# NVIDIA-Merlin/distributed-embeddings

Measured on AMD Instinct MI355X. Metric: samples/sec (whole node) DLRM-Criteo-1TB bs/gpu=65536, higher is better.
Workload: dtype bf16; 1 GPU; model=DLRM-Criteo-1TB, global_batch=65536, batch_per_gpu=65536, embedding_dim=128, parallelism=hybrid dp+mp (strategy=memory_balanced) x1

## Files before the change

distributed_embeddings_amd/csrc/dot_interact.hip:

```cpp

#include <hip/hip_runtime.h>
#include <hip/hip_bf16.h>

#include "ops_api.h"

#define WAVE 64

typedef __attribute__((ext_vector_type(8))) short bf16x8;
typedef __attribute__((ext_vector_type(4))) float f32x4;


template <int FMAX>
__global__ void dot_interact_fwd(const __hip_bfloat16* __restrict__ feats,
                                 __hip_bfloat16* __restrict__ out, int64_t B,
                                 int F, int D, int out_w, int tri_n) {
  extern __shared__ short lds_all[];
  const int wave = threadIdx.x >> 6;
  const int lane = threadIdx.x & (WAVE - 1);
  const int ldst = D + 8;
  short* lds = lds_all + wave * FMAX * ldst;
  const int64_t n_waves = ((int64_t)gridDim.x * blockDim.x) >> 6;
  const int64_t wave_id = ((int64_t)blockIdx.x * blockDim.x + threadIdx.x) >> 6;

  for (int64_t b = wave_id; b < B; b += n_waves) {
    const short* src = reinterpret_cast<const short*>(feats) + b * (int64_t)F * D;
    const int total8 = FMAX * D / 8;
    for (int i = lane; i < total8; i += WAVE) {
      const int elem = i * 8;
      const int row = elem / D, col = elem % D;
      if (elem < F * D) {
        *reinterpret_cast<bf16x8*>(&lds[row * ldst + col]) =
            *reinterpret_cast<const bf16x8*>(&src[elem]);
      } else {
        bf16x8 z = {0, 0, 0, 0, 0, 0, 0, 0};
        *reinterpret_cast<bf16x8*>(&lds[row * ldst + col]) = z;
      }
    }

    const int r16 = lane & 15;
    const int khalf = lane >> 4;

    const int tiles_mi[3] = {0, 1, 1};
    const int tiles_ni[3] = {0, 0, 1};
#pragma unroll
    for (int t = 0; t < 3; ++t) {
      const int mi = tiles_mi[t], ni = tiles_ni[t];
      f32x4 acc = {0.f, 0.f, 0.f, 0.f};
      for (int k0 = 0; k0 < D; k0 += 32) {
        bf16x8 a = *reinterpret_cast<const bf16x8*>(
            &lds[(mi * 16 + r16) * ldst + k0 + khalf * 8]);
        bf16x8 bfr = *reinterpret_cast<const bf16x8*>(
            &lds[(ni * 16 + r16) * ldst + k0 + khalf * 8]);
        acc = __builtin_amdgcn_mfma_f32_16x16x32_bf16(a, bfr, acc, 0, 0, 0);
      }
      __hip_bfloat16* orow = out + b * (int64_t)out_w;
#pragma unroll
      for (int reg = 0; reg < 4; ++reg) {
        const int i = mi * 16 + (lane >> 4) * 4 + reg;
        const int j = ni * 16 + (lane & 15);
        if (i > j && i < F && j < F) {
          orow[i * (i - 1) / 2 + j] = __hip_bfloat16(acc[reg]);
        }
      }
    }
    short* orow_s = reinterpret_cast<short*>(out + b * (int64_t)out_w);
    for (int c = lane; c < D; c += WAVE) {
      orow_s[tri_n + c] = lds[c];
    }
    for (int c = tri_n + D + lane; c < out_w; c += WAVE) {
      orow_s[c] = 0;
    }
  }
}

template <int FMAX>
__global__ void dot_interact_bwd(const __hip_bfloat16* __restrict__ gout,
                                 const __hip_bfloat16* __restrict__ feats,
                                 __hip_bfloat16* __restrict__ gfeats, int64_t B,
                                 int F, int D, int out_w, int tri_n) {
  extern __shared__ short lds_all[];
  const int wave = threadIdx.x >> 6;
  const int lane = threadIdx.x & (WAVE - 1);
  short* lds = lds_all + wave * (FMAX * D + FMAX * FMAX);
  short* gsym = lds + FMAX * D;
  const int64_t n_waves = ((int64_t)gridDim.x * blockDim.x) >> 6;
  const int64_t wave_id = ((int64_t)blockIdx.x * blockDim.x + threadIdx.x) >> 6;

  for (int64_t b = wave_id; b < B; b += n_waves) {
    const short* src = reinterpret_cast<const short*>(feats) + b * (int64_t)F * D;
    const int total8 = FMAX * D / 8;
    for (int i = lane; i < total8; i += WAVE) {
      const int elem = i * 8;
      if (elem < F * D) {
        *reinterpret_cast<bf16x8*>(&lds[elem]) =
            *reinterpret_cast<const bf16x8*>(&src[elem]);
      } else {
        bf16x8 z = {0, 0, 0, 0, 0, 0, 0, 0};
        *reinterpret_cast<bf16x8*>(&lds[elem]) = z;
      }
    }
    const __hip_bfloat16* grow = gout + b * (int64_t)out_w;
    for (int idx = lane; idx < FMAX * FMAX; idx += WAVE) {
      const int i = idx / FMAX, j = idx % FMAX;
      float g = 0.f;
      if (i < F && j < F && i != j) {
        const int r = i > j ? i : j, c = i > j ? j : i;
        g = float(grow[r * (r - 1) / 2 + c]);
      }
      __hip_bfloat16 hb(g);
      gsym[idx] = *reinterpret_cast<short*>(&hb);
    }

    const int r16 = lane & 15;
    const int khalf = lane >> 4;
    __hip_bfloat16* gf = gfeats + b * (int64_t)F * D;

    for (int nj = 0; nj < D / 16; ++nj) {
#pragma unroll
      for (int mi = 0; mi < FMAX / 16; ++mi) {
        f32x4 acc = {0.f, 0.f, 0.f, 0.f};
#pragma unroll
        for (int k0 = 0; k0 < FMAX; k0 += 32) {
          bf16x8 a = *reinterpret_cast<const bf16x8*>(
              &gsym[(mi * 16 + r16) * FMAX + k0 + khalf * 8]);
          bf16x8 bfr;
#pragma unroll
          for (int r = 0; r < 8; ++r) {
            bfr[r] = lds[(k0 + khalf * 8 + r) * D + nj * 16 + r16];
          }
          acc = __builtin_amdgcn_mfma_f32_16x16x32_bf16(a, bfr, acc, 0, 0, 0);
        }
#pragma unroll
        for (int reg = 0; reg < 4; ++reg) {
          const int i = mi * 16 + (lane >> 4) * 4 + reg;
          const int j = nj * 16 + (lane & 15);
          if (i < F && j < D) {
            float v = acc[reg];
            if (i == 0) v += float(grow[tri_n + j]);
            gf[i * D + j] = __hip_bfloat16(v);
          }
        }
      }
    }
  }
}



static int di_wpb(int dflt) {
  static int v = [] {
    const char* e = getenv("DE_DI_WPB");
    if (!e) return 0;
    int i = atoi(e);
    return (i == 2 || i == 4 || i == 8) ? i : 0;
  }();
  return v ? v : dflt;
}

template <int FMAX, int WPB>
__global__ void dot_interact_fwd_packed(
    const __hip_bfloat16* __restrict__ bottom,
    const __hip_bfloat16* __restrict__ packed,
    const int* __restrict__ perm, __hip_bfloat16* __restrict__ out, int64_t B,
    int F, int D, int out_w, int tri_n, int64_t sb, int64_t sp) {
  extern __shared__ short lds_all[];
  const int wave = threadIdx.x >> 6;
  const int lane = threadIdx.x & (WAVE - 1);
  const int tid = threadIdx.x;
  const int ldst = D + 8;
  short* lds = lds_all + wave * FMAX * ldst;
  const int d8 = D / 8;

  for (int64_t b0 = (int64_t)blockIdx.x * WPB; b0 < B;
       b0 += (int64_t)gridDim.x * WPB) {
    for (int i = tid; i < FMAX * WPB * d8; i += WPB * WAVE) {
      const int row = i / (WPB * d8);
      const int rem = i % (WPB * d8);
      const int w = rem / d8;
      const int col = (rem % d8) * 8;
      const int64_t b = b0 + w;
      bf16x8 v = {0, 0, 0, 0, 0, 0, 0, 0};
      if (b < B) {
        if (row == 0) {
          v = *reinterpret_cast<const bf16x8*>(
              reinterpret_cast<const short*>(bottom) + b * (int64_t)D + col);
        } else if (row < F) {
          v = *reinterpret_cast<const bf16x8*>(
              reinterpret_cast<const short*>(packed) +
              ((int64_t)perm[row - 1] * sp + b * sb) * (int64_t)D + col);
        }
      }
      *reinterpret_cast<bf16x8*>(
          &lds_all[w * FMAX * ldst + row * ldst + col]) = v;
    }
    __syncthreads();

    const int64_t b = b0 + wave;
    if (b < B) {
      const int r16 = lane & 15;
      const int khalf = lane >> 4;
      const int tiles_mi[3] = {0, 1, 1};
      const int tiles_ni[3] = {0, 0, 1};
#pragma unroll
      for (int t = 0; t < 3; ++t) {
        const int mi = tiles_mi[t], ni = tiles_ni[t];
        f32x4 acc = {0.f, 0.f, 0.f, 0.f};
        for (int k0 = 0; k0 < D; k0 += 32) {
          bf16x8 a = *reinterpret_cast<const bf16x8*>(
              &lds[(mi * 16 + r16) * ldst + k0 + khalf * 8]);
          bf16x8 bfr = *reinterpret_cast<const bf16x8*>(
              &lds[(ni * 16 + r16) * ldst + k0 + khalf * 8]);
          acc = __builtin_amdgcn_mfma_f32_16x16x32_bf16(a, bfr, acc, 0, 0, 0);
        }
        __hip_bfloat16* orow = out + b * (int64_t)out_w;
#pragma unroll
        for (int reg = 0; reg < 4; ++reg) {
          const int i = mi * 16 + (lane >> 4) * 4 + reg;
          const int j = ni * 16 + (lane & 15);
          if (i > j && i < F && j < F) {
            orow[i * (i - 1) / 2 + j] = __hip_bfloat16(acc[reg]);
          }
        }
      }
      short* orow_s = reinterpret_cast<short*>(out + b * (int64_t)out_w);
      for (int c = lane; c < D; c += WAVE) {
        orow_s[tri_n + c] = lds[c];
      }
      for (int c = tri_n + D + lane; c < out_w; c += WAVE) {
        orow_s[c] = 0;
      }
    }
    __syncthreads();
  }
}

template <int FMAX, int WPB>
__global__ void dot_interact_bwd_packed(
    const __hip_bfloat16* __restrict__ gout,
    const __hip_bfloat16* __restrict__ bottom,
    const __hip_bfloat16* __restrict__ packed, const int* __restrict__ perm,
    __hip_bfloat16* __restrict__ gbottom, __hip_bfloat16* __restrict__ gpacked,
    int64_t B, int F, int D, int out_w, int tri_n, int64_t sb, int64_t sp) {
  extern __shared__ short lds_all[];
  const int wave = threadIdx.x >> 6;
  const int lane = threadIdx.x & (WAVE - 1);
  const int tid = threadIdx.x;
  const int per_wave = FMAX * D + FMAX * FMAX;
  short* lds = lds_all + wave * per_wave;
  short* gsym = lds + FMAX * D;
  const int d8 = D / 8;

  for (int64_t b0 = (int64_t)blockIdx.x * WPB; b0 < B;
       b0 += (int64_t)gridDim.x * WPB) {
    for (int i = tid; i < FMAX * WPB * d8; i += WPB * WAVE) {
      const int row = i / (WPB * d8);
      const int rem = i % (WPB * d8);
      const int w = rem / d8;
      const int col = (rem % d8) * 8;
      const int64_t b = b0 + w;
      bf16x8 v = {0, 0, 0, 0, 0, 0, 0, 0};
      if (b < B) {
        if (row == 0) {
          v = *reinterpret_cast<const bf16x8*>(
              reinterpret_cast<const short*>(bottom) + b * (int64_t)D + col);
        } else if (row < F) {
          v = *reinterpret_cast<const bf16x8*>(
              reinterpret_cast<const short*>(packed) +
              ((int64_t)perm[row - 1] * sp + b * sb) * (int64_t)D + col);
        }
      }
      *reinterpret_cast<bf16x8*>(
          &lds_all[w * per_wave + row * D + col]) = v;
    }
    __syncthreads();

    const int64_t b = b0 + wave;
    if (b < B) {
      const __hip_bfloat16* grow = gout + b * (int64_t)out_w;
      for (int idx = lane; idx < FMAX * FMAX; idx += WAVE) {
        const int i = idx / FMAX, j = idx % FMAX;
        float g = 0.f;
        if (i < F && j < F && i != j) {
          const int r = i > j ? i : j, c = i > j ? j : i;
          g = float(grow[r * (r - 1) / 2 + c]);
        }
        __hip_bfloat16 hb(g);
        gsym[idx] = *reinterpret_cast<short*>(&hb);
      }

      const int r16 = lane & 15;
      const int khalf = lane >> 4;
      for (int nj = 0; nj < D / 16; ++nj) {
        f32x4 accs[FMAX / 16];
#pragma unroll
        for (int mi = 0; mi < FMAX / 16; ++mi) {
          f32x4 acc = {0.f, 0.f, 0.f, 0.f};
#pragma unroll
          for (int k0 = 0; k0 < FMAX; k0 += 32) {
            bf16x8 a = *reinterpret_cast<const bf16x8*>(
                &gsym[(mi * 16 + r16) * FMAX + k0 + khalf * 8]);
            bf16x8 bfr;
#pragma unroll
            for (int r = 0; r < 8; ++r) {
              bfr[r] = lds[(k0 + khalf * 8 + r) * D + nj * 16 + r16];
            }
            acc = __builtin_amdgcn_mfma_f32_16x16x32_bf16(a, bfr, acc, 0, 0, 0);
          }
          accs[mi] = acc;
        }
#pragma unroll
        for (int mi = 0; mi < FMAX / 16; ++mi) {
#pragma unroll
          for (int reg = 0; reg < 4; ++reg) {
            const int i = mi * 16 + (lane >> 4) * 4 + reg;
            const int j = nj * 16 + (lane & 15);
            float v = accs[mi][reg];
            if (i == 0) v += float(grow[tri_n + j]);
            __hip_bfloat16 hb(v);
            lds[i * D + j] = *reinterpret_cast<short*>(&hb);
          }
        }
      }
    }
    __syncthreads();

    for (int i = tid; i < FMAX * WPB * d8; i += WPB * WAVE) {
      const int row = i / (WPB * d8);
      const int rem = i % (WPB * d8);
      const int w = rem / d8;
      const int col = (rem % d8) * 8;
      const int64_t b = b0 + w;
      if (b >= B || row >= F) continue;
      const bf16x8 v = *reinterpret_cast<const bf16x8*>(
          &lds_all[w * per_wave + row * D + col]);
      if (row == 0) {
        *reinterpret_cast<bf16x8*>(
            reinterpret_cast<short*>(gbottom) + b * (int64_t)D + col) = v;
      } else {
        *reinterpret_cast<bf16x8*>(
            reinterpret_cast<short*>(gpacked) +
            ((int64_t)perm[row - 1] * sp + b * sb) * (int64_t)D + col) = v;
      }
    }
    __syncthreads();
  }
}

void launch_dot_interact_fwd_packed(const void* bottom, const void* packed,
                                    const int* perm, void* out, int64_t B,
                                    int F, int D, int out_w, int tri_n,
                                    int64_t sb, int64_t sp,
                                    hipStream_t stream) {
  const int wpb = di_wpb(2);
  const int block = wpb * WAVE;
  int64_t blocks = (B + wpb - 1) / wpb;
  if (blocks > 32768) blocks = 32768;
  const size_t lds = (size_t)wpb * 32 * (D + 8) * sizeof(short);
#define LFWD(W)                                                                \
  hipLaunchKernelGGL((dot_interact_fwd_packed<32, W>), dim3((int)blocks),      \
                     dim3(block), lds, stream,                                 \
                     (const __hip_bfloat16*)bottom,                            \
                     (const __hip_bfloat16*)packed, perm, (__hip_bfloat16*)out,\
                     B, F, D, out_w, tri_n, sb, sp)
  if (wpb == 2) LFWD(2); else if (wpb == 8) LFWD(8); else LFWD(4);
#undef LFWD
}

void launch_dot_interact_bwd_packed(const void* gout, const void* bottom,
                                    const void* packed, const int* perm,
                                    void* gbottom, void* gpacked, int64_t B,
                                    int F, int D, int out_w, int tri_n,
                                    int64_t sb, int64_t sp,
                                    hipStream_t stream) {
  const int wpb = di_wpb(8);
  const int block = wpb * WAVE;
  int64_t blocks = (B + wpb - 1) / wpb;
  if (blocks > 32768) blocks = 32768;
  const size_t lds = (size_t)wpb * (32 * D + 32 * 32) * sizeof(short);
#define LBWD(W)                                                                \
  hipLaunchKernelGGL((dot_interact_bwd_packed<32, W>), dim3((int)blocks),      \
                     dim3(block), lds, stream, (const __hip_bfloat16*)gout,    \
                     (const __hip_bfloat16*)bottom,                            \
                     (const __hip_bfloat16*)packed, perm,                      \
                     (__hip_bfloat16*)gbottom, (__hip_bfloat16*)gpacked, B, F, \
                     D, out_w, tri_n, sb, sp)
  if (wpb == 2) LBWD(2); else if (wpb == 8) LBWD(8); else LBWD(4);
#undef LBWD
}

void launch_dot_interact_fwd(const void* feats, void* out, int64_t B, int F,
                             int D, int out_w, int tri_n, hipStream_t stream) {
  const int block = 256;
  const int waves = block / WAVE;
  int64_t blocks = (B + waves - 1) / waves;
  if (blocks > 8192) blocks = 8192;
  const size_t lds = (size_t)waves * 32 * (D + 8) * sizeof(short);
  hipLaunchKernelGGL((dot_interact_fwd<32>), dim3((int)blocks), dim3(block),
                     lds, stream, (const __hip_bfloat16*)feats,
                     (__hip_bfloat16*)out, B, F, D, out_w, tri_n);
}

void launch_dot_interact_bwd(const void* gout, const void* feats, void* gfeats,
                             int64_t B, int F, int D, int out_w, int tri_n,
                             hipStream_t stream) {
  const int block = 256;
  const int waves = block / WAVE;
  int64_t blocks = (B + waves - 1) / waves;
  if (blocks > 8192) blocks = 8192;
  const size_t lds = (size_t)waves * (32 * D + 32 * 32) * sizeof(short);
  hipLaunchKernelGGL((dot_interact_bwd<32>), dim3((int)blocks), dim3(block),
                     lds, stream, (const __hip_bfloat16*)gout,
                     (const __hip_bfloat16*)feats, (__hip_bfloat16*)gfeats, B,
                     F, D, out_w, tri_n);
}
```

Baseline: 16.32 million samples/s.

## Specialize packed dot-interaction kernels on compile-time embedding dim with MFMA tile restructuring

Adds D-templated forward and backward packed dot-interaction kernels, used when D is 32, 64, 128 or 256. They precompute gather offsets per thread, launch one block per group instead of grid-striding, and compute only the three needed lower-triangular 16x16 tiles in forward. Forward stages each output row in LDS so it can be written with vectorized stores. Backward uses swizzled LDS, transposed LDS reads (ds_read_tr16) and per-wave fences in place of block barriers. Default waves per block change to 4 for both directions. The cost is added code complexity, larger register use from the unrolled offset arrays, and a fallback path only for unsupported D.

```diff
diff --git a/distributed_embeddings_amd/csrc/dot_interact.hip b/distributed_embeddings_amd/csrc/dot_interact.hip
--- a/distributed_embeddings_amd/csrc/dot_interact.hip
+++ b/distributed_embeddings_amd/csrc/dot_interact.hip
@@ -147,6 +147,8 @@
 
 
 
+#define DI_WPB_FWD 4
+#define DI_WPB_BWD 4
 static int di_wpb(int dflt) {
   static int v = [] {
     const char* e = getenv("DE_DI_WPB");
@@ -158,7 +160,7 @@
 }
 
 template <int FMAX, int WPB>
-__global__ void dot_interact_fwd_packed(
+__global__ void dot_interact_fwd_packed_rt(
     const __hip_bfloat16* __restrict__ bottom,
     const __hip_bfloat16* __restrict__ packed,
     const int* __restrict__ perm, __hip_bfloat16* __restrict__ out, int64_t B,
@@ -235,7 +237,7 @@
 }
 
 template <int FMAX, int WPB>
-__global__ void dot_interact_bwd_packed(
+__global__ void dot_interact_bwd_packed_rt(
     const __hip_bfloat16* __restrict__ gout,
     const __hip_bfloat16* __restrict__ bottom,
     const __hip_bfloat16* __restrict__ packed, const int* __restrict__ perm,
@@ -346,23 +348,355 @@
   }
 }
 
+
+typedef __attribute__((ext_vector_type(4))) short bf16x4;
+typedef bf16x8 __attribute__((aligned(2))) bf16x8_u;
+typedef short v4i16_t __attribute__((vector_size(8)));
+typedef __attribute__((address_space(3))) v4i16_t lds_v4i16_t;
+
+__device__ __forceinline__ void wave_lds_fence() {
+  __builtin_amdgcn_fence(__ATOMIC_ACQ_REL, "wavefront");
+  __builtin_amdgcn_wave_barrier();
+}
+
+__device__ __forceinline__ short f32_to_bf16_bits(float v) {
+  __hip_bfloat16 hb(v);
+  return *reinterpret_cast<short*>(&hb);
+}
+
+__device__ __forceinline__ float bf16_bits_to_f32(short s) {
+  return __builtin_bit_cast(float, (unsigned)(unsigned short)s << 16);
+}
+
+template <int D>
+__device__ __forceinline__ int swz(int row, int col) {
+  const int sw = (((row & 3) << 2) | ((row >> 2) & 3)) & (D / 8 - 1);
+  return row * D + ((((col >> 3) ^ sw) << 3) | (col & 7));
+}
+
+template <int D, int WPB>
+struct PackedIO {
+  static constexpr int D8 = D / 8;
+  static constexpr int RPI = WAVE / D8;
+  static constexpr int NIT = 32 / RPI;
+  int r0, w, col;
+  int64_t b;
+  int64_t off[NIT];
+
+  __device__ __forceinline__ PackedIO(const int* __restrict__ perm, int F,
+                                      int64_t b0, int64_t sb, int64_t sp) {
+    const int tid = threadIdx.x;
+    r0 = tid / (WPB * D8);
+    w = (tid / D8) % WPB;
+    col = (tid % D8) * 8;
+    b = b0 + w;
+    int prow[NIT];
+#pragma unroll
+    for (int it = 0; it < NIT; ++it) {
+      const int row = it * RPI + r0;
+      const int pi = row < 1 ? 0 : (row < F ? row - 1 : F - 2);
+      prow[it] = perm[pi];
+    }
+#pragma unroll
+    for (int it = 0; it < NIT; ++it) {
+      const int row = it * RPI + r0;
+      off[it] = row == 0 ? b * D + col
+                         : (prow[it] * sp + b * sb) * (int64_t)D + col;
+    }
+#pragma unroll
+    for (int it = 0; it < NIT; ++it) asm volatile("" : "+v"(off[it]));
+  }
+
+  template <int LD, int PER_WAVE, bool SWZ>
+  __device__ __forceinline__ void load(const short* __restrict__ bottom,
+                                       const short* __restrict__ packed,
+                                       short* lds_all, int64_t B, int F) const {
+    bf16x8 v[NIT];
+#pragma unroll
+    for (int it = 0; it < NIT; ++it) {
+      const int row = it * RPI + r0;
+      const bf16x8 z = {0, 0, 0, 0, 0, 0, 0, 0};
+      v[it] = z;
+      if (b < B && row < F) {
+        v[it] = *reinterpret_cast<const bf16x8*>(
+            (row == 0 ? bottom : packed) + off[it]);
+      }
+    }
+#pragma unroll
+    for (int it = 0; it < NIT; ++it) {
+      const int row = it * RPI + r0;
+      const int at_lds = SWZ ? swz<D>(row, col) : row * LD + col;
+      *reinterpret_cast<bf16x8*>(&lds_all[w * PER_WAVE + at_lds]) = v[it];
+    }
+  }
+};
+
+template <int D, int WPB>
+__global__ __launch_bounds__(WPB* WAVE) void dot_interact_fwd_packed(
+    const __hip_bfloat16* __restrict__ bottom,
+    const __hip_bfloat16* __restrict__ packed,
+    const int* __restrict__ perm, __hip_bfloat16* __restrict__ out, int64_t B,
+    int F, int out_w, int tri_n, int64_t sb, int64_t sp) {
+  extern __shared__ short lds_all[];
+  constexpr int LD = D + 8;
+  constexpr int PER_WAVE = 32 * LD;
+  const int wave = __builtin_amdgcn_readfirstlane(threadIdx.x >> 6);
+  const int lane = threadIdx.x & (WAVE - 1);
+  short* lds = lds_all + wave * PER_WAVE;
+  const int64_t b0 = (int64_t)blockIdx.x * WPB;
+  const PackedIO<D, WPB> io(perm, F, b0, sb, sp);
+  {
+    io.template load<LD, PER_WAVE, false>(
+        reinterpret_cast<const short*>(bottom),
+        reinterpret_cast<const short*>(packed), lds_all, B, F);
+    __syncthreads();
+
+    const int64_t b = b0 + wave;
+    if (b < B) {
+      const int r16 = lane & 15;
+      const int khalf = lane >> 4;
+      const int tiles_mi[3] = {0, 1, 1};
+      const int tiles_ni[3] = {0, 0, 1};
+      f32x4 accs[3];
+#pragma unroll
+      for (int t = 0; t < 3; ++t) {
+        const int mi = tiles_mi[t], ni = tiles_ni[t];
+        f32x4 acc = {0.f, 0.f, 0.f, 0.f};
+#pragma unroll
+        for (int k0 = 0; k0 < D; k0 += 32) {
+          bf16x8 a = *reinterpret_cast<const bf16x8*>(
+              &lds[(mi * 16 + r16) * LD + k0 + khalf * 8]);
+          bf16x8 bfr = *reinterpret_cast<const bf16x8*>(
+              &lds[(ni * 16 + r16) * LD + k0 + khalf * 8]);
+          acc = __builtin_amdgcn_mfma_f32_16x16x32_bf16(a, bfr, acc, 0, 0, 0);
+        }
+        accs[t] = acc;
+      }
+      wave_lds_fence();
+      short* stage = lds + LD;
+#pragma unroll
+      for (int t = 0; t < 3; ++t) {
+#pragma unroll
+        for (int reg = 0; reg < 4; ++reg) {
+          const int i = tiles_mi[t] * 16 + khalf * 4 + reg;
+          const int j = tiles_ni[t] * 16 + r16;
+          if (i > j && i < F) {
+            stage[i * (i - 1) / 2 + j] = f32_to_bf16_bits(accs[t][reg]);
+          }
+        }
+      }
+#pragma unroll
+      for (int c = lane; c < D; c += WAVE) stage[tri_n + c] = lds[c];
+      const int width = tri_n + D;
+      const int width8 = (width + 7) & ~7;
+      if (width + lane < width8) stage[width + lane] = 0;
+      wave_lds_fence();
+
+      short* orow = reinterpret_cast<short*>(out) + b * (int64_t)out_w;
+      const int nfull = out_w >> 3;
+      for (int c = lane; c < nfull; c += WAVE) {
+        bf16x8 v = {0, 0, 0, 0, 0, 0, 0, 0};
+        if (c * 8 < width8) v = *reinterpret_cast<const bf16x8*>(&stage[c * 8]);
+        *reinterpret_cast<bf16x8_u*>(&orow[c * 8]) = v;
+      }
+      const int e = nfull * 8 + lane;
+      if (e < out_w) orow[e] = e < width ? stage[e] : (short)0;
+    }
+    __syncthreads();
+  }
+}
+
+template <int D, int WPB>
+__global__ __launch_bounds__(WPB* WAVE, D >= 256 ? 2 : 4) void
+dot_interact_bwd_packed(
+    const __hip_bfloat16* __restrict__ gout,
+    const __hip_bfloat16* __restrict__ bottom,
+    const __hip_bfloat16* __restrict__ packed, const int* __restrict__ perm,
+    __hip_bfloat16* __restrict__ gbottom, __hip_bfloat16* __restrict__ gpacked,
+    int64_t B, int F, int out_w, int tri_n, int64_t sb, int64_t sp) {
+  static_assert(496 + 7 + D <= 1024, "gout row staging needs D <= 256");
+  extern __shared__ short lds_all[];
+  constexpr int PER_WAVE = 32 * D + 1024;
+  constexpr int D8 = D / 8;
+  constexpr int NJ = D / 16;
+  using IO = PackedIO<D, WPB>;
+  const int wave = __builtin_amdgcn_readfirstlane(threadIdx.x >> 6);
+  const int lane = threadIdx.x & (WAVE - 1);
+  short* lds = lds_all + wave * PER_WAVE;
+  short* stage = lds + 32 * D;
+  short* gb = stage + 1024 - D;
+  const int64_t b0 = (int64_t)blockIdx.x * WPB;
+  const IO io(perm, F, b0, sb, sp);
+  {
+    const int64_t b = b0 + wave;
+    const bf16x8 z = {0, 0, 0, 0, 0, 0, 0, 0};
+    bf16x8 vt = z, vb = z;
+    if (b < B) {
+      const short* grow = reinterpret_cast<const short*>(gout) +
+                          b * (int64_t)out_w;
+      if (lane * 8 < tri_n) {
+        vt = *reinterpret_cast<const bf16x8_u*>(&grow[lane * 8]);
+      }
+      if (lane < D8) {
+        vb = *reinterpret_cast<const bf16x8_u*>(&grow[tri_n + lane * 8]);
+      }
+    }
+    io.template load<D, PER_WAVE, true>(
+        reinterpret_cast<const short*>(bottom),
+        reinterpret_cast<const short*>(packed), lds_all, B, F);
+    if (b < B) {
+      if (lane * 8 < tri_n) *reinterpret_cast<bf16x8*>(&stage[lane * 8]) = vt;
+      if (lane < D8) *reinterpret_cast<bf16x8*>(&gb[lane * 8]) = vb;
+    }
+    __syncthreads();
+
+    if (b < B) {
+      const int r16 = lane & 15;
+      const int khalf = lane >> 4;
+      bf16x8 g[2];
+#pragma unroll
+      for (int ni = 0; ni < 2; ++ni) {
+#pragma unroll
+        for (int j = 0; j < 8; ++j) {
+          const int i = ni * 16 + r16, k = khalf * 8 + j;
+          const bool ok = i < F && k < F && i != k;
+          const int r = i > k ? i : k, c = i > k ? k : i;
+          const short s = stage[ok ? r * (r - 1) / 2 + c : 0];
+          g[ni][j] = ok ? s : (short)0;
+        }
+      }
+      const int xrow = khalf * 8 + (r16 >> 2), xcol = (lane & 3) * 4;
+      constexpr int NJB = NJ < 4 ? NJ : 4;
+#pragma unroll
+      for (int nj0 = 0; nj0 < NJ; nj0 += NJB) {
+        bf16x8 a[NJB];
+        bf16x4 gbv[NJB];
+#pragma unroll
+        for (int t = 0; t < NJB; ++t) {
+          const int d0 = (nj0 + t) * 16;
+          const v4i16_t lo = __builtin_amdgcn_ds_read_tr16_b64_v4i16(
+              (lds_v4i16_t*)(lds + swz<D>(xrow, d0 + xcol)));
+          const v4i16_t hi = __builtin_amdgcn_ds_read_tr16_b64_v4i16(
+              (lds_v4i16_t*)(lds + swz<D>(xrow + 4, d0 + xcol)));
+          a[t] = bf16x8{lo[0], lo[1], lo[2], lo[3], hi[0], hi[1], hi[2], hi[3]};
+          gbv[t] = *reinterpret_cast<const bf16x4*>(&gb[d0 + khalf * 4]);
+        }
+        wave_lds_fence();
+#pragma unroll
+        for (int t = 0; t < NJB; ++t) {
+          const int d0 = (nj0 + t) * 16;
+          f32x4 c0 = {0.f, 0.f, 0.f, 0.f};
+          if (r16 == 0) {
+#pragma unroll
+            for (int reg = 0; reg < 4; ++reg) {
+              c0[reg] = bf16_bits_to_f32(gbv[t][reg]);
+            }
+          }
+          const f32x4 zc = {0.f, 0.f, 0.f, 0.f};
+          const f32x4 acc0 =
+              __builtin_amdgcn_mfma_f32_16x16x32_bf16(a[t], g[0], c0, 0, 0, 0);
+          const f32x4 acc1 =
+              __builtin_amdgcn_mfma_f32_16x16x32_bf16(a[t], g[1], zc, 0, 0, 0);
+          const bf16x4 o0 = {
+              f32_to_bf16_bits(acc0[0]), f32_to_bf16_bits(acc0[1]),
+              f32_to_bf16_bits(acc0[2]), f32_to_bf16_bits(acc0[3])};
+          const bf16x4 o1 = {
+              f32_to_bf16_bits(acc1[0]), f32_to_bf16_bits(acc1[1]),
+              f32_to_bf16_bits(acc1[2]), f32_to_bf16_bits(acc1[3])};
+          *reinterpret_cast<bf16x4*>(&lds[swz<D>(r16, d0 + khalf * 4)]) = o0;
+          *reinterpret_cast<bf16x4*>(
+              &lds[swz<D>(16 + r16, d0 + khalf * 4)]) = o1;
+        }
+        wave_lds_fence();
+      }
+    }
+    __syncthreads();
+
+    {
+      const int64_t bw = io.b;
+      bf16x8 v[IO::NIT];
+#pragma unroll
+      for (int it = 0; it < IO::NIT; ++it) {
+        const int row = it * IO::RPI + io.r0;
+        v[it] = *reinterpret_cast<const bf16x8*>(
+            &lds_all[io.w * PER_WAVE + swz<D>(row, io.col)]);
+      }
+#pragma unroll
+      for (int it = 0; it < IO::NIT; ++it) {
+        const int row = it * IO::RPI + io.r0;
+        if (bw < B && row < F) {
+          short* dst = reinterpret_cast<short*>(row == 0 ? gbottom : gpacked);
+          *reinterpret_cast<bf16x8*>(dst + io.off[it]) = v[it];
+        }
+      }
+    }
+    __syncthreads();
+  }
+}
+
+#define DI_FOR_WPB(M) \
+  if (wpb == 2) { M(2); } else if (wpb == 8) { M(8); } else { M(4); }
+
+template <int D>
+static void launch_fwd_packed_d(const void* bottom, const void* packed,
+                                const int* perm, void* out, int64_t B, int F,
+                                int out_w, int tri_n, int64_t sb, int64_t sp,
+                                int wpb, int blocks, hipStream_t stream) {
+  const size_t lds = (size_t)wpb * 32 * (D + 8) * sizeof(short);
+#define LFWD(W)                                                                \
+  hipLaunchKernelGGL((dot_interact_fwd_packed<D, W>), dim3(blocks),            \
+                     dim3(W * WAVE), lds, stream,                              \
+                     (const __hip_bfloat16*)bottom,                            \
+                     (const __hip_bfloat16*)packed, perm, (__hip_bfloat16*)out,\
+                     B, F, out_w, tri_n, sb, sp)
+  DI_FOR_WPB(LFWD)
+#undef LFWD
+}
+
+template <int D>
+static void launch_bwd_packed_d(const void* gout, const void* bottom,
+                                const void* packed, const int* perm,
+                                void* gbottom, void* gpacked, int64_t B, int F,
+                                int out_w, int tri_n, int64_t sb, int64_t sp,
+                                int wpb, int blocks, hipStream_t stream) {
+  const size_t lds = (size_t)wpb * (32 * D + 32 * 32) * sizeof(short);
+#define LBWD(W)                                                                \
+  hipLaunchKernelGGL((dot_interact_bwd_packed<D, W>), dim3(blocks),            \
+                     dim3(W * WAVE), lds, stream, (const __hip_bfloat16*)gout, \
+                     (const __hip_bfloat16*)bottom,                            \
+                     (const __hip_bfloat16*)packed, perm,                      \
+                     (__hip_bfloat16*)gbottom, (__hip_bfloat16*)gpacked, B, F, \
+                     out_w, tri_n, sb, sp)
+  DI_FOR_WPB(LBWD)
+#undef LBWD
+}
+
 void launch_dot_interact_fwd_packed(const void* bottom, const void* packed,
                                     const int* perm, void* out, int64_t B,
                                     int F, int D, int out_w, int tri_n,
                                     int64_t sb, int64_t sp,
                                     hipStream_t stream) {
-  const int wpb = di_wpb(2);
-  const int block = wpb * WAVE;
-  int64_t blocks = (B + wpb - 1) / wpb;
-  if (blocks > 32768) blocks = 32768;
+  const int wpb = di_wpb(DI_WPB_FWD);
+  const int64_t groups = (B + wpb - 1) / wpb;
+  const bool fixed_ok = groups <= INT32_MAX && F >= 2;
+  int blocks = (int)groups;
+#define LFWD_D(DD)                                                             \
+  launch_fwd_packed_d<DD>(bottom, packed, perm, out, B, F, out_w, tri_n, sb,   \
+                          sp, wpb, blocks, stream)
+  if (fixed_ok && D == 128) { LFWD_D(128); return; }
+  if (fixed_ok && D == 64) { LFWD_D(64); return; }
+  if (fixed_ok && D == 32) { LFWD_D(32); return; }
+  if (fixed_ok && D == 256) { LFWD_D(256); return; }
+#undef LFWD_D
+  if (groups > 32768) blocks = 32768;
   const size_t lds = (size_t)wpb * 32 * (D + 8) * sizeof(short);
 #define LFWD(W)                                                                \
-  hipLaunchKernelGGL((dot_interact_fwd_packed<32, W>), dim3((int)blocks),      \
-                     dim3(block), lds, stream,                                 \
+  hipLaunchKernelGGL((dot_interact_fwd_packed_rt<32, W>), dim3(blocks),        \
+                     dim3(W * WAVE), lds, stream,                              \
                      (const __hip_bfloat16*)bottom,                            \
                      (const __hip_bfloat16*)packed, perm, (__hip_bfloat16*)out,\
                      B, F, D, out_w, tri_n, sb, sp)
-  if (wpb == 2) LFWD(2); else if (wpb == 8) LFWD(8); else LFWD(4);
+  DI_FOR_WPB(LFWD)
 #undef LFWD
 }
 
@@ -372,21 +706,31 @@
                                     int F, int D, int out_w, int tri_n,
                                     int64_t sb, int64_t sp,
                                     hipStream_t stream) {
-  const int wpb = di_wpb(8);
-  const int block = wpb * WAVE;
-  int64_t blocks = (B + wpb - 1) / wpb;
-  if (blocks > 32768) blocks = 32768;
+  const int wpb = di_wpb(DI_WPB_BWD);
+  const int64_t groups = (B + wpb - 1) / wpb;
+  const bool fixed_ok = groups <= INT32_MAX && F >= 2;
+  int blocks = (int)groups;
+#define LBWD_D(DD)                                                             \
+  launch_bwd_packed_d<DD>(gout, bottom, packed, perm, gbottom, gpacked, B, F,  \
+                          out_w, tri_n, sb, sp, wpb, blocks, stream)
+  if (fixed_ok && D == 128) { LBWD_D(128); return; }
+  if (fixed_ok && D == 64) { LBWD_D(64); return; }
+  if (fixed_ok && D == 32) { LBWD_D(32); return; }
+  if (fixed_ok && D == 256) { LBWD_D(256); return; }
+#undef LBWD_D
+  if (groups > 32768) blocks = 32768;
   const size_t lds = (size_t)wpb * (32 * D + 32 * 32) * sizeof(short);
 #define LBWD(W)                                                                \
-  hipLaunchKernelGGL((dot_interact_bwd_packed<32, W>), dim3((int)blocks),      \
-                     dim3(block), lds, stream, (const __hip_bfloat16*)gout,    \
+  hipLaunchKernelGGL((dot_interact_bwd_packed_rt<32, W>), dim3(blocks),        \
+                     dim3(W * WAVE), lds, stream, (const __hip_bfloat16*)gout, \
                      (const __hip_bfloat16*)bottom,                            \
                      (const __hip_bfloat16*)packed, perm,                      \
                      (__hip_bfloat16*)gbottom, (__hip_bfloat16*)gpacked, B, F, \
                      D, out_w, tri_n, sb, sp)
-  if (wpb == 2) LBWD(2); else if (wpb == 8) LBWD(8); else LBWD(4);
+  DI_FOR_WPB(LBWD)
 #undef LBWD
 }
+#undef DI_FOR_WPB
 
 void launch_dot_interact_fwd(const void* feats, void* out, int64_t B, int F,
                              int D, int out_w, int tri_n, hipStream_t stream) {
```

New measurement: 17.71 million samples/s (median of 6 runs). +8.5%, better.
